# HKUST-Aerial-Robotics/VINS-Mono

Measured on AMD Instinct MI355X. Metric: sliding-window BA solves/sec (Estimator::optimization: 8-iteration dogleg solve + marginalization), higher is better.
Workload: dtype f64; 1 GPU; batch of 256 independent EuRoC-shape windows per step and GPU (K=11 frames, ~150 landmarks, 10 IMU factors, ~600 projection factors, 75-dim marginalization prior, max 8 iterations, MARGIN_OLD marginalization); windows resident in HBM; consecutive steps are issued to 16 HIP streams (independent batches in flight); windows_per_gpu=256, batches_in_flight=16, parallelism=independent batches x1 (no collectives)

## Files before the change

vins-mono_amd/csrc/ba_host.hip:

```cpp
#include "vg_range.h"
#include <hip/hip_runtime.h>
#include <algorithm>
#include <chrono>
#include <cmath>
#include <cstdio>
#include <cstdlib>
#include <cstring>
#include <string>
#include <thread>
#include <vector>
#include "ba_layout.h"
#include "vg_handle.h"
#include "../../include/vinsgpu.h"

struct BaFork { hipStream_t aux; hipEvent_t fork, join; };
extern "C" hipError_t ba_launch_solve(const BaLayout& L, const BaLayout* dL, const BaPtrs& P, int rounds, hipStream_t stream,
                                      hipEvent_t* ev, int* kinds, int* n_launches, const BaFork* fk);
typedef int (*BaAllReduce)(void* user, double* buf, size_t count, void* stream);
extern "C" hipError_t ba_launch_solve_big(const BaLayout& L, const BaLayout* dL, const BaPtrs& P, int rounds, int slack, hipStream_t stream,
                                          BaAllReduce allreduce, void* user, int* hook_rc, hipEvent_t* ev, int* kinds, int* n_launches);
extern "C" hipError_t ba_launch_eval_factors(const BaLayout& L, const BaLayout* dL, const BaPtrs& P, double* proj_r, double* proj_J,
                                            double* imu_r, double* imu_J, double* prior_r, hipStream_t stream);
extern "C" const char* ba_failed_launch();
extern "C" hipError_t ba_prepare_launch();
// ... 215 lines not shown
        else { L.l_pmap = 0; L.l_pinv = o; o += up(L.R, 4) / 2; }
        if (L.big) { L.l_di = o; o += up(L.Rc + 1, 2); L.l_cz = o; o += 6 * 96; }
        L.l_Sg = 0;
        if (L.big) { L.l_Sg = oo; oo += up((L.Rc + 1) * (L.Rc + 2) / 2, 2); }
        L.lds_solve = o * 8;
        bigm_doubles = ob;
        if (!L.big && L.Rc + 10 - 64 > 32) { h->err = "solve kernel: more column tasks than three wavefronts"; return VG_ERR_UNSUPPORTED; }
        if (!L.big && 36 * ldc < std::max(std::max(L.RcPad * 33, 2 * SV_NT), std::max(9 * L.K, 162))) { h->err = "solve kernel: scratch does not fit the coupling-row ring"; return VG_ERR_UNSUPPORTED; }
        if (L.lds_solve > 160 * 1024) { h->err = "solve kernel LDS carve exceeds 160 KB"; return VG_ERR_UNSUPPORTED; }
        const int nib = std::min(std::min(L.K - 1, BA_IMU_BATCH), L.igs);
        L.lds_lin = 8 * std::max(up(nib * 225, 2) + nib * 480, 5 * L.Ncap);
        L.lds_pro = 8 * BA_NW * (L.imu_info ? 512 : 256);
        if (8 * L.Ncap * L.Ncap <= 128 * 1024) L.lds_pro = std::max(L.lds_pro, 8 * L.Ncap * L.Ncap);
        if (L.lds_lin > 128 * 1024) { h->err = "prior too large for the linearisation kernel"; return VG_ERR_UNSUPPORTED; }
        {
            static const bool env_off = getenv("VG_BA_FUSED") && !strcmp(getenv("VG_BA_FUSED"), "0");
            const bool off = env_off && !h->ba.no_env;
            static const int env_min = getenv("VG_BA_FUSED_MIN") ? atoi(getenv("VG_BA_FUSED_MIN")) : 32;
            const int la_min_windows = h->ba.fused_min >= 0 ? (h->ba.fused_min ? h->ba.fused_min : 1 << 30) : (env_min ? env_min : 1 << 30);
            const int npair = L.Kp * (L.Kp - 1) / 2;
            const int avail = (160 * 1024 - 8192 - 512) / 8;
            const int nstl = up(7 * L.Kp + 9 * L.K + 8, 2);
            int chf = (int)((avail - nstl - npair * 90 - 34 - (64 + 82 + 8 * 80) / 2) / 34.0);
            chf = std::min(chf & ~1, 512);
            L.la_on = (!off && L.nwin >= la_min_windows && !L.big && !L.e && !L.t && L.Kp <= 13 && chf >= 96 && (L.Fcap + chf - 17) / (chf - 16) <= 62) ? 1 : 0;
            L.la_chf = chf; L.la_chq = chf - 16;
            L.la_P = up(chf * 33, 2);
            L.la_key = L.la_P + up(npair * 90, 2);
            L.la_x = up(L.la_key + (2 * chf + 64 + 82 + 8 * 80 + 1) / 2 + 2, 2);
            L.lds_linacc = (L.la_x + nstl) * 8;
        }
        {
            static const int env_max = getenv("VG_BA_SOLVE_W8_BELOW") ? atoi(getenv("VG_BA_SOLVE_W8_BELOW")) : -1;
            const int below = (env_max >= 0 && !h->ba.no_env) ? env_max : 32;
            L.sv_w8 = (!L.big && L.nwin < below) ? 1 : 0;
            L.l_wd8 = L.lds_solve / 8;
            L.lds_solve_w8 = L.lds_solve + 8 * L.RcPad * 33;
            if (L.lds_solve_w8 > 160 * 1024) L.sv_w8 = 0;
        }
    }
    if (L.big) {
        const int nt = (L.Rc + 1 + 15) / 16;
        L.nts = nt * (nt + 1) / 2;
        const int ntri = L.Rc * (L.Rc + 1) / 2;
        L.rb1_T = up(ntri + L.Rc, 2);
        L.rb1_scal = L.rb1_T + up((L.Rc + 1) * (L.Rc + 2) / 2, 2);
        L.rb1_len = L.rb1_scal + RB1_NSCAL;
    }
    int o = 0;
    L.io_hdr = o; o += BA_HDR_INTS;
    L.io_lm_start = o; o += L.Lcap;
    L.io_lm_fbeg = o; o += L.Lcap + 8;
    L.io_fac_i = o; o += L.Fcap;
// ... 42 lines not shown
    L.so_gn = o; o += L.Rpad + L.Lcap;
    L.so_yl = o; o += L.Lcap;
    L.so_lsc = o; o += L.Lcap;
    L.so_xp = 0;
    if (!L.big) { L.so_xp = o; o += up(9 * L.K, 4) * L.ldc; }
    if (L.big) {
        L.so_bigm = o; o += up(bigm_doubles, 8);
        L.so_dgl = o; o += 2 * L.Lcap;
        L.so_gtl = o; o += 2 * L.Lcap;
    }
    {
        int b = 0;
        L.bo_Sp = b; b += up(L.Rc * (L.Rc + 1) / 2, 2);
        L.bo_gp = b; b += L.RcPad;
        L.bo_h = b; b += L.Lcap;
        L.bo_b = b; b += L.Lcap;
        L.bo_Wt = b; b += L.RcPad * L.Lcap;
        L.bo_imuJ = b; b += (L.K - 1) * 512;
        L.bo_pr = b; b += L.Ncap;
        L.bo_gpr = b; b += L.Ncap;
        L.buf_stride = up(b, 8);
    }
    L.so_buf = o; o += 2 * L.buf_stride;
    L.sstride = up(o, 8);
    L.pl_off = (int)((sizeof(BaLayout) + 255) / 256 * 256);
    L.pl_n = L.big ? 0 : L.Rc * (L.Rc + 1) / 2 + L.Rpad + 2 * 81 * L.K;
    o = 0;
    L.oo_pose = o; o += up(7 * L.Kp, 2);
    L.oo_sb = o; o += up(9 * L.K, 2);
    L.oo_ex = o; o += 8;
    L.oo_td = o; o += 2;
    L.oo_lam = o; o += L.Lcap;
    L.oo_sum = o; o += BA_SUM_DOUBLES;
    L.oo_trace = o; o += 5 * VG_MAX_ITERS + 16;
    L.ostride = up(o, 8);
    L.oi_stride = up(4 + VG_MAX_ITERS, 8);
    L.mcap = up(6 * L.K + 9 * 2 + 6 + 1, 8);
    if (L.mcap > 256) { h->err = "kept dimension of the marginalization beyond the kernel's tables"; return VG_ERR_UNSUPPORTED; }
    const int mcap = L.mcap;
    L.mo_J0 = 0;
    L.mo_r0 = mcap * mcap;
    L.mo_x0 = L.mo_r0 + mcap;
    L.mo_stride = up(L.mo_x0 + (L.K + 4) * 9, 8);
    L.mi_stride = up(8 + 2 * (L.K + 4) + 16, 8);
    L.mg_posmax = up(mcap + 15 + L.Lcap, 2);
    {
// ... 1144 lines not shown
```

vins-mono_amd/csrc/ba_layout.h:

```cpp
#pragma once

#ifndef BA_NT
#define BA_NT 512
#endif
#define BA_NW (BA_NT / 64)
#ifndef SV_NT
#define SV_NT 256
#endif
#define SV_NW (SV_NT / 64)
#define SV_WG_PER_CU (SV_NT <= 256 ? 2 : 1)
#define BA_LIN_NT 256
#define BA_ACC_NT 256
#define BA_MAX_K 13
#define BA_MAX_K_LARGE 40
#define BA_MARG_LDS_INTS 400
#ifndef BA_IMU_BATCH
#define BA_IMU_BATCH 16
#endif
#ifndef BA_IMU_GROUP
#define BA_IMU_GROUP 2
#endif
#define BA_IMU_STRIDE 472
#define BA_OBS_STRIDE 8
#define BA_SUM_DOUBLES 16
#define BA_HDR_INTS 16

enum { H_L = 0, H_F, H_NPRIOR, H_NBLK, H_MAXIT, H_NCHUNK, H_MARGIN, H_STATUS, H_MARGMODE };

enum {
    C_IT = 0, C_NACC, C_NINV, C_TERM, C_STATUS, C_RADIUS, C_MU, C_MUSOLVED, C_REUSE, C_COST, C_XNORM, C_ALPHA, C_GTN2,
    C_GNN2, C_GTGN, C_DNORM, C_MODEL, C_CUR, C_PENDING, C_DONE, C_STEPNORM, C_XNORMC, C_INITCOST, C_SCALED, C_QCAM,
    C_PHASE, C_GNN2C, C_GTGNC, C_STEP2C, C_XN2C,
    C_T0,
    C_TIMEDOUT,
    C_NCTL = 32
};

enum { RB1_COST = 0, RB1_GTL2, RB1_LAM2, RB1_STEP2, RB1_NBIG, RB1_NSCAL = 8 };
enum { RB2_GNN2 = 0, RB2_GTGN, RB2_QL, RB2_NONFIN };
#define BA_BIG_LM_BLOCKS 32
#define BA_BIG_ZERO_BLOCKS 8
#define RB2_LEN (4 * BA_BIG_LM_BLOCKS)

enum { V_G = 0, V_SC, V_DG, V_GT, V_GN, V_U, V_Y, V_T, V_DI, V_NVEC };
struct alignas(16) AsmPlanEntry { int dst, base, imu, cols; };

struct BaLayout {
    int nwin, K, Kp, e, t;
// ... 8 lines not shown
        io_pair_ptr, io_task_list, io_imu_valid, io_pb_kind, io_pb_idx, io_pb_col, io_pb_off, io_pb_x0off, istride;
    int do_pose, do_sb, do_ex, do_td, do_lam, do_obs, do_imu, do_par, dstride;
    int po_x0, po_r0, po_J0, pld, pstride;
    int so_ctl, so_part, so_x, so_lam;
    int so_imuU, so_Hp, so_rec;
    int so_J0t;
    int so_sc, so_sl, so_dg, so_gt, so_gn;
    int so_yl, so_lsc;
    int so_xp;
    int so_buf, buf_stride;
    int bo_Sp, bo_gp, bo_h, bo_b, bo_Wt, bo_imuJ, bo_pr, bo_gpr;
    int sstride;
    int oo_pose, oo_sb, oo_ex, oo_td, oo_lam, oo_sum, oo_trace, ostride;
    int oi_stride;
    int mo_J0, mo_r0, mo_x0, mo_stride;
    int mi_stride;
    int ms_stride;
    int mcap, mg_ld, mg_posmax, mg_cs, mg_lds_bytes;
    int l_S, l_XC, l_D, l_E, l_dinv, l_vec, l_red, l_wd, l_z, l_pmap, ldc, lds_solve;
    int l_ring, l_pinv;
    int pl_off, pl_n;
    int lds_lin, lds_pro;
    int la_on, la_chq, la_chf, la_P, la_key, la_x, lds_linacc;
    int sv_w8;
    int l_wd8, lds_solve_w8;
    int pro_split;
    int big;
    int so_bigm;
    int l_di, l_cz;
    int l_Sg;
    int so_dgl, so_gtl;
    int rb1_len, rb1_T, rb1_scal;
    int nts;
};

struct BaPtrs {
    int* iarr;
    double* din;
    double* scr;
    double* out;
    int* iout;
    double* mout;
    int* miout;
    double* mscr;
    double* rb1;
    double* rb2;
// ... 5 lines not shown
```

vins-mono_amd/csrc/ba_pipeline.hip:

```cpp
#include <hip/hip_runtime.h>
#include <vector>
#include <mutex>
#include <cstring>
#include <cstdlib>
#include "ba_layout.h"
#include "ba_factors.h"
#include "../../include/vinsgpu.h"

extern __shared__ __attribute__((aligned(16))) char bp_smem[];

#ifdef BA_SOLVE_W8_TU
#undef BA_PROFILE_DETAIL
#undef BA_DEBUG_DUMP
namespace vg_w8 {
#endif

#define NOINL __device__ __noinline__
#define AS_LDS(p) ((lds_d*)(p))
#define AS_LDS_C(p) ((const lds_d*)(p))
#define AS_GLB(p) ((glb_d*)(p))
#define AS_GLB_C(p) ((const glb_d*)(p))
#define AS_GLB_CI(p) ((const glb_i*)(p))
template <bool BIG> struct MovT { typedef lds_d D; typedef lds_i I; };
template <> struct MovT<true> { typedef glb_d D; typedef glb_i I; };
// ... 43 lines not shown
    for (int k_ = c.tid; k_ < L.lds_solve / 8; k_ += SV_NT) g_dbg[(slot) * DBG_SLOT + k_] = LDSB[k_]; \
    if ((slot) >= 2) for (int k_ = c.tid; k_ < 9 * L.K * L.ldc; k_ += SV_NT) g_dbg[5 * DBG_SLOT + k_] = m.xp[k_]; \
    __syncthreads(); } } while (0)
#else
#define DBG_DUMP(slot)
#endif
enum { PF_JUDGE = 0, PF_ASM, PF_DG, PF_BUILD, PF_CHAIN, PF_SCHUR, PF_CHOL, PF_BACK, PF_CBACK, PF_LMY, PF_NORMS, PF_CAND, PF_TAIL };


struct Ctx {
    const BaLayout* Lp;
    const int* hdr;
    const int* ia;
    const double* di;
    const double* pri;
    double* sc;
    int tid, lane, wave;
    int nL, nF, nprior, nblk;
    double focal, tr, row, gnorm;
};

DEV BaLayout layout_load(const BaLayout* Lp) { return const_load(Lp); }

DEV void ctx_init(Ctx& c, const BaLayout* Lp, const BaPtrs& P, int w) {
    const BaLayout L = layout_load(Lp);
    c.Lp = Lp;
    c.ia = P.iarr + (size_t)w * L.istride;
    c.hdr = c.ia + L.io_hdr;
    c.di = P.din + (size_t)w * L.dstride;
    c.sc = P.scr + (size_t)w * L.sstride;
    c.pri = P.pri + (size_t)w * L.pstride;
    c.tid = threadIdx.x; c.lane = c.tid & 63; c.wave = c.tid >> 6;
    c.nL = uni(c.hdr[H_L]); c.nF = uni(c.hdr[H_F]); c.nprior = uni(c.hdr[H_NPRIOR]); c.nblk = uni(c.hdr[H_NBLK]);
    c.focal = uni(c.di[L.do_par + P_FOCAL]); c.tr = uni(c.di[L.do_par + P_TR]); c.row = uni(c.di[L.do_par + P_ROW]);
    c.gnorm = uni(c.di[L.do_par + P_GNORM]);
}

DEV double block_sum(double* red, int nw, int lane, int wave, double v) {
    v = wave_sum_all(v);
    __syncthreads();
    if (lane == 0) red[wave] = v;
    __syncthreads();
    double s = 0.0;
    for (int w = 0; w < nw; ++w) s += red[w];
    return uni(s);
}
DEV void block_sum2(double* red, int nw, int lane, int wave, double& a, double& b) {
    a = wave_sum_all(a);
    b = wave_sum_all(b);
    __syncthreads();
    if (lane == 0) { red[wave] = a; red[nw + wave] = b; }
    __syncthreads();
    double s = 0.0, t = 0.0;
    for (int w = 0; w < nw; ++w) { s += red[w]; t += red[nw + w]; }
// ... 207 lines not shown
#pragma unroll
            for (int k = 0; k < 15; ++k) A[c.lane * 15 + k] = a[k];
        }
        __builtin_amdgcn_wave_barrier();
        glb_d* Uo = AS_GLB(c.sc + L.so_imuU + f * 225);
        if (c.lane < 15) {
            const int j = c.lane;
            double x[15];
#pragma unroll
            for (int i = 14; i >= 0; --i) {
                double s = (i == j) ? 1.0 : 0.0;
#pragma unroll
                for (int k = 14; k > i; --k) s -= (k <= j) ? A[i * 15 + k] * x[k] : 0.0;
                x[i] = (i <= j) ? s / A[i * 15 + i] : 0.0;
            }
#pragma unroll
            for (int i = 0; i < 15; ++i) Uo[i * 15 + j] = x[i];
        }
        __builtin_amdgcn_wave_barrier();
    }
    __syncthreads();
}

#ifndef BA_SOLVE_W8_TU
extern "C" __global__ __launch_bounds__(BA_NT) void ba_prologue_kernel(const BaLayout* __restrict__ Lp, BaPtrs P) {
    const BaLayout& L = *Lp;
    Ctx c;
    ctx_init(c, Lp, P, blockIdx.x);
    double* x = c.sc + L.so_x;
    DP_DECL;
    const bool all = gridDim.y == 1;
    const int part = blockIdx.y, nI = (L.K - 1 + BA_NW - 1) / BA_NW;
    if (all || part == 0)
    {
        double* out = P.out + (size_t)blockIdx.x * L.ostride;
        int* iout = P.iout + (size_t)blockIdx.x * L.oi_stride;
        int* miout = P.miout + (size_t)blockIdx.x * L.mi_stride;
        for (int k = c.tid; k < L.ostride; k += BA_NT) out[k] = 0.0;
        for (int k = c.tid; k < L.oi_stride; k += BA_NT) iout[k] = 0;
        for (int k = c.tid; k < L.mi_stride; k += BA_NT) miout[k] = 0;
    }
    if (all || part == 0) {
        for (int k = c.tid; k < 7 * L.Kp; k += BA_NT) x[k] = c.di[L.do_pose + k];
        for (int k = c.tid; k < 9 * L.K; k += BA_NT) x[7 * L.Kp + k] = c.di[L.do_sb + k];
        if (c.tid < 7) x[7 * L.Kp + 9 * L.K + c.tid] = c.di[L.do_ex + c.tid];
        if (c.tid == 7) x[7 * L.Kp + 9 * L.K + 7] = c.di[L.do_td];
        for (int k = c.tid; k < c.nL; k += BA_NT) c.sc[L.so_lam + k] = c.di[L.do_lam + k];
        if (c.tid < C_NCTL) {
            double v = 0.0;
            if (c.tid == C_RADIUS) v = 1e4;
            if (c.tid == C_MU || c.tid == C_MUSOLVED) v = 1e-8;
            if (c.tid == C_T0) v = (double)wall_clock64();
            c.sc[L.so_ctl + c.tid] = v;
        }
    }
    DP_ADD(40);
    if (all || (part >= 1 && part <= nI)) {
        const int fbeg = all ? 0 : (part - 1) * BA_NW, fend = all ? L.K - 1 : part * BA_NW;
        if (L.imu_info) imu_sqrt_info_ref(c, fbeg, fend);
        else imu_sqrt_info(c, fbeg, fend);
    }
    DP_ADD(41);
    if (c.nprior && (all || part > nI)) {
        const bool do_copy = all || part == nI + 1, do_prod = all || part == nI + 2;
        const int n = c.nprior;
        const double* J0 = c.pri + L.po_J0;
        double* Hp = c.sc + L.so_Hp;
        if (do_copy) {
            double* J0t = c.sc + L.so_J0t;
            for (int wk = c.tid; wk < n * n; wk += BA_NT) { const int r = wk / n, cc = wk % n; J0t[cc * L.Ncap + r] = J0[r * L.pld + cc]; }
        }
        __syncthreads();
        DP_ADD(42);
        if (!do_prod) {
        } else if ((size_t)n * n * 8 <= (size_t)L.lds_pro) {
            double* J0s = LDSB;
            for (int wk = c.tid; wk < n * n; wk += BA_NT) J0s[wk] = J0[(wk / n) * L.pld + wk % n];
// ... 292 lines not shown
struct ProjIn {
    double pi[7], pj[7], oi[8], oj[8], ex[8];
    double lam;
    int i, j, l;
};
DEV void proj_fetch(const Ctx& c, int f, const double* x_, const double* lam_, ProjIn& p) {
    const BaLayout& L = *c.Lp;
    const glb_i* ia = AS_GLB_CI(c.ia);
    const glb_d* x = AS_GLB_C(x_);
    const glb_d* obs = AS_GLB_C(c.di + L.do_obs);
    p.i = ia[L.io_fac_i + f];
    p.j = ia[L.io_fac_j + f];
    p.l = ia[L.io_fac_lm + f];
    const int oi = ia[L.io_fac_oi + f], oj = ia[L.io_fac_oj + f];
#pragma unroll
    for (int k = 0; k < 7; ++k) { p.pi[k] = x[7 * p.i + k]; p.pj[k] = x[7 * p.j + k]; }
#pragma unroll
    for (int k = 0; k < 8; ++k) {
        p.oi[k] = obs[oi * BA_OBS_STRIDE + k];
        p.oj[k] = obs[oj * BA_OBS_STRIDE + k];
        p.ex[k] = x[7 * L.Kp + 9 * L.K + k];
    }
    p.lam = AS_GLB_C(lam_)[p.l];
}
DEV void proj_fetch_staged(const Ctx& c, int f, const lds_d* xs, const double* lam_, ProjIn& p) {
    const BaLayout& L = *c.Lp;
    const glb_i* ia = AS_GLB_CI(c.ia);
    const glb_d* obs = AS_GLB_C(c.di + L.do_obs);
    p.i = ia[L.io_fac_i + f];
    p.j = ia[L.io_fac_j + f];
    p.l = ia[L.io_fac_lm + f];
    const int oi = ia[L.io_fac_oi + f], oj = ia[L.io_fac_oj + f];
#pragma unroll
    for (int k = 0; k < 8; ++k) {
        p.oi[k] = obs[oi * BA_OBS_STRIDE + k];
        p.oj[k] = obs[oj * BA_OBS_STRIDE + k];
    }
    p.lam = AS_GLB_C(lam_)[p.l];
#pragma unroll
    for (int k = 0; k < 7; ++k) { p.pi[k] = xs[7 * p.i + k]; p.pj[k] = xs[7 * p.j + k]; }
#pragma unroll
    for (int k = 0; k < 8; ++k) p.ex[k] = xs[7 * L.Kp + 9 * L.K + k];
}
DEV void proj_jac(const Ctx& c, const ProjIn& p, double* r, double* Ji, double* Jj, double* Jex,
                  double* Jl, double* Jtd) {
    const BaLayout& L = *c.Lp;
    if (L.t) {
        if (L.e) proj_eval<true, true, true>(p.pi, p.pj, p.ex, p.lam, p.oi, p.oj, p.ex[7], c.focal, c.tr, c.row, r, Ji, Jj, Jex, Jl, Jtd);
        else proj_eval<true, true, false>(p.pi, p.pj, p.ex, p.lam, p.oi, p.oj, p.ex[7], c.focal, c.tr, c.row, r, Ji, Jj, Jex, Jl, Jtd);
    } else {
        if (L.e) proj_eval<false, true, true>(p.pi, p.pj, p.ex, p.lam, p.oi, p.oj, 0.0, c.focal, c.tr, c.row, r, Ji, Jj, Jex, Jl, Jtd);
        else proj_eval<false, true, false>(p.pi, p.pj, p.ex, p.lam, p.oi, p.oj, 0.0, c.focal, c.tr, c.row, r, Ji, Jj, Jex, Jl, Jtd);
    }
}

NOINL double proj_linearize(const Ctx& c_in, int f, const double* x, const double* lam, double* recs) {
    const Ctx c = c_in;
    const BaLayout L = *c.Lp;
    ProjIn p;
    proj_fetch(c, f, x, lam, p);
    double r[2], Ji[12], Jj[12], Jex[12], Jl[2], Jtd[2];
    proj_jac(c, p, r, Ji, Jj, Jex, Jl, Jtd);
    const double s = r[0] * r[0] + r[1] * r[1];
    const double sq = sqrt(1.0 / (1.0 + s));
    glb_d* rec = AS_GLB(recs) + (size_t)AS_GLB_CI(c.ia)[L.io_fac_slot + f] * L.REC;
// ... 260 lines not shown
    const int bx = rest % L.nba, w = (rest / L.nba) * 8 + xcd;
    if (w >= L.nwin) return;
    Ctx c;
    ctx_init(c, Lp, P, w);
    const double* ctl = c.sc + L.so_ctl;
    if (ctl[C_DONE] != 0.0) return;
    const int which = ((int)ctl[C_CUR]) ^ (ctl[C_PENDING] != 0.0 ? 1 : 0);
    double* buf = lin_buf(c, which);
    const double* recs = c.sc + L.so_rec;
    __shared__ double part[7 * 36 + 4];
    if (bx < L.Kp) { diag_pose_task(c, bx, recs, buf + L.bo_Sp, buf + L.bo_gp, part); return; }
    const int ng = L.e + L.t;
    if (ng && bx == L.Kp) { global_task(c, recs, buf + L.bo_Sp, buf + L.bo_gp, part); return; }
    const int g = (bx - L.Kp - (ng ? 1 : 0)) * (BA_ACC_NT / 64) + c.wave;
    const int nother = L.ntask - L.Kp - ng * (ng + 1) / 2;
    if (g < nother) owner_task(c, c.ia[L.io_task_list + g], c.lane, recs, buf + L.bo_Sp, buf + L.bo_gp);
    else {
        const int l = (g - nother) * 64 + c.lane;
        if (l < L.Lcap) landmark_task(c, l, recs, buf);
    }
}
#endif

#define LA_NT BA_NT
#define LA_RS 33
#define LA_NPW 6
#define LA_MAXP 13
#define LA_QCAP 80
static_assert(LA_QCAP <= 128, "the pair prefix of ba_linacc_proj_kernel takes two pairs per lane of one wavefront");
#define LA_PAIR 90
DEV int wave_scan_incl(int v) {
    v += __builtin_amdgcn_update_dpp(0, v, 0x111, 0xF, 0xF, true);
    v += __builtin_amdgcn_update_dpp(0, v, 0x112, 0xF, 0xF, true);
    v += __builtin_amdgcn_update_dpp(0, v, 0x114, 0xF, 0xF, true);
    v += __builtin_amdgcn_update_dpp(0, v, 0x118, 0xF, 0xF, true);
    const int r0 = __builtin_amdgcn_readlane(v, 15), r1 = __builtin_amdgcn_readlane(v, 31), r2 = __builtin_amdgcn_readlane(v, 47);
    const int row = (int)(threadIdx.x & 63) >> 4;
    return v + (row > 0 ? r0 : 0) + (row > 1 ? r1 : 0) + (row > 2 ? r2 : 0);
}
DEV int la_pair_q(int i, int j, int Kp) { const int d = j - i; return (d - 1) * Kp - (d - 1) * d / 2 + i; }
__device__ __forceinline__ void linacc_body(const BaLayout* __restrict__ Lp, const BaPtrs& P) {
    const BaLayout L = layout_load(Lp);
    Ctx c;
    ctx_init(c, Lp, P, blockIdx.x);
    const double* ctl = c.sc + L.so_ctl;
    if (ctl[C_DONE] != 0.0) return;
    const int which = uni(((int)ctl[C_CUR]) ^ (ctl[C_PENDING] != 0.0 ? 1 : 0));
    const double* x = c.sc + L.so_x + which * L.nst;
    const double* lam = c.sc + L.so_lam + which * L.Lcap;
    glb_d* buf = AS_GLB(lin_buf(c, which));
    const glb_i* ia = AS_GLB_CI(c.ia);
    lds_d* rec = AS_LDS(LDSB);
    lds_d* Pb = AS_LDS(LDSB + L.la_P);
    lds_i* key = (lds_i*)(LDSB + L.la_key);
    lds_i* lstart = key + L.la_chf;
    lds_i* posx = lstart + 64;
    lds_i* pstart = posx + L.la_chf;
    lds_i* wcnt = pstart + LA_QCAP + 2;
    __shared__ double red[2 * (LA_NT / 64)];
    const int Kp = L.Kp, npair = Kp * (Kp - 1) / 2, chq = L.la_chq;
    const int nL = c.nL;
    DP_DECL;
    {
        double share = 0.0;
        if (c.nprior > 0) {
            if (c.nprior * c.nprior <= 12 * LA_NT && 4 * L.Ncap <= 4 * LA_NT && (c.nprior * (c.nprior + 1) + 2 + 5 * L.Ncap) <= L.la_P)
                share = prior_staged(c, L, x, lin_buf(c, which) + L.bo_pr, lin_buf(c, which) + L.bo_gpr, LDSB);
            else
                share = prior_pass(c, x, lin_buf(c, which) + L.bo_pr, lin_buf(c, which) + L.bo_gpr, LDSB);
        }
        DP_ADD(23);
        share += imu_pass<true>(c, x, lin_buf(c, which) + L.bo_imuJ, 0, L.K - 1);
        const double tot_imu = block_sum(red, LA_NT / 64, c.lane, c.wave, share);
        for (int g = c.tid; g < L.nbl - L.nbf; g += LA_NT) c.sc[L.so_part + L.nbf + g] = g == 0 ? tot_imu : 0.0;
        __syncthreads();
        DP_ADD(22);
    }
    lds_d* xs = AS_LDS(LDSB + L.la_x);
    for (int k = c.tid; k < 7 * L.Kp + 9 * L.K + 8; k += LA_NT) xs[k] = AS_GLB_C(x)[k];
    const int nchunk = nL > 0 ? uni(ia[L.io_lm_fbeg + nL - 1] / chq + 1) : 0;
    for (int t = c.tid; t < nL; t += LA_NT) {
        const int cl = ia[L.io_lm_fbeg + t] / chq;
        if (t == 0 || ia[L.io_lm_fbeg + t - 1] / chq != cl) lstart[cl] = t;
    }
    if (c.tid == 0) lstart[nchunk] = nL;
    for (int e = c.tid; e < npair * LA_PAIR; e += LA_NT) Pb[e] = 0.0;
    const bool pair_wave = c.wave < LA_NPW;
    __syncthreads();
    DP_ADD(24);
    int pidx[4];
#pragma unroll
    for (int reg = 0; reg < 4; ++reg) {
        const int row = (c.lane >> 4) + 4 * reg, col = c.lane & 15;
        int idx = -1;
        if (row < 6) {
            if (col <= row) idx = row * (row + 1) / 2 + col;
            else if (col == 13) idx = 78 + row;
        } else if (row < 12) {
            if (col < 6) idx = 42 + (row - 6) * 6 + col;
            else if (col <= row && col < 12) idx = 21 + (row - 6) * (row - 5) / 2 + (col - 6);
            else if (col == 13) idx = 84 + (row - 6);
        }
        pidx[reg] = idx;
    }
    double cost = 0.0;
    for (int ch = 0; ch < nchunk; ++ch) {
        const int l0 = lstart[ch], l1 = lstart[ch + 1];
        const int f0 = ia[L.io_lm_fbeg + l0], f1 = ia[L.io_lm_fbeg + l1];
        const int nf = uni(f1 - f0);
        if (nf > L.la_chf) __builtin_trap();
        ProjIn pin;
        int q = -1, rank = 0;
        if (c.tid < nf) {
            proj_fetch_staged(c, f0 + c.tid, xs, lam, pin);
            q = la_pair_q(pin.i, pin.j, Kp);
        }
        for (int e = c.tid; e < (LA_NT / 64) * LA_QCAP; e += LA_NT) wcnt[e] = 0;
        __syncthreads();
        DP_ADD(45);
        {
            const unsigned long long act = __ballot(q >= 0);
            unsigned long long same = act;
#pragma unroll
            for (int b = 0; b < 7; ++b) {
                const bool bit = q >= 0 && ((q >> b) & 1);
                const unsigned long long mb = __ballot(bit);
                same &= bit ? mb : ~mb;
            }
            const unsigned long long lt = (1ull << c.lane) - 1ull;
            rank = __popcll(same & lt);
            if (q >= 0 && rank == 0) wcnt[c.wave * LA_QCAP + q] = __popcll(same);
        }
        __syncthreads();
        if (c.wave == 0) {
            int cw0[LA_NT / 64], cw1[LA_NT / 64];
            const int p0 = c.lane, p1 = c.lane + 64;
#pragma unroll
            for (int w = 0; w < LA_NT / 64; ++w) {
                cw0[w] = p0 < npair ? wcnt[w * LA_QCAP + p0] : 0;
                cw1[w] = p1 < npair ? wcnt[w * LA_QCAP + p1] : 0;
            }
            int t0 = 0, t1 = 0;
#pragma unroll
            for (int w = 0; w < LA_NT / 64; ++w) { const int a = cw0[w], b = cw1[w]; cw0[w] = t0; cw1[w] = t1; t0 += a; t1 += b; }
            const int i0 = wave_scan_incl(t0);
            const int tot0 = __builtin_amdgcn_readlane(i0, 63);
            const int i1 = wave_scan_incl(t1) + tot0;
            if (p0 < npair) {
                pstart[p0 + 1] = i0;
#pragma unroll
                for (int w = 0; w < LA_NT / 64; ++w) wcnt[w * LA_QCAP + p0] = i0 - t0 + cw0[w];
            }
            if (p1 < npair) {
                pstart[p1 + 1] = i1;
#pragma unroll
                for (int w = 0; w < LA_NT / 64; ++w) wcnt[w * LA_QCAP + p1] = i1 - t1 + cw1[w];
            }
            if (c.lane == 0) pstart[0] = 0;
        }
        __syncthreads();
        DP_ADD(46);
        if (c.tid < nf) {
            const int pos = wcnt[c.wave * LA_QCAP + q] + rank;
            double r[2], Ji[12], Jj[12], Jl[2];
            proj_eval<false, true, false>(pin.pi, pin.pj, pin.ex, pin.lam, pin.oi, pin.oj, 0.0, c.focal, c.tr, c.row, r, Ji, Jj, nullptr, Jl, nullptr);
            const double s = r[0] * r[0] + r[1] * r[1];
            const double sq = sqrt(1.0 / (1.0 + s));
            lds_d* qr = rec + pos * LA_RS;
#pragma unroll
            for (int k = 0; k < 6; ++k) {
                qr[k] = sq * Ji[k]; qr[16 + k] = sq * Ji[6 + k];
                qr[6 + k] = sq * Jj[k]; qr[22 + k] = sq * Jj[6 + k];
            }
            qr[12] = sq * Jl[0]; qr[28] = sq * Jl[1];
            qr[13] = sq * r[0]; qr[29] = sq * r[1];
            key[c.tid] = pin.i * 16 + pin.j;
            posx[c.tid] = pos;
            cost += log1p(s);
        }
        __syncthreads();
        DP_ADD(25);
        if (pair_wave) {
            double4_t acc[LA_MAXP];
#pragma unroll
            for (int k = 0; k < LA_MAXP; ++k) acc[k] = (double4_t){0, 0, 0, 0};
            const int k4 = c.lane >> 4, col = c.lane & 15;
            const int xo = (k4 & 1) * 16 + col;
            const int hi = k4 >> 1;
            const bool incol = col < 14;
#pragma unroll
            for (int k = 0; k < LA_MAXP; ++k) {
                const int qk = c.wave + LA_NPW * k;
                if (qk >= npair) continue;
                const int pb0 = uni(pstart[qk]), pe0 = uni(pstart[qk + 1]);
                DP_ADD(29);
                for (int e = pb0; e < pe0; e += 4) {
                    const int f0r = e + hi, f1r = e + 2 + hi;
                    const double v0 = (f0r < pe0 && incol) ? rec[f0r * LA_RS + xo] : 0.0;
                    const double v1 = (f1r < pe0 && incol) ? rec[f1r * LA_RS + xo] : 0.0;
                    acc[k] = __builtin_amdgcn_mfma_f64_16x16x4f64(v0, v0, acc[k], 0, 0, 0);
                    if (e + 2 < pe0) acc[k] = __builtin_amdgcn_mfma_f64_16x16x4f64(v1, v1, acc[k], 0, 0, 0);
                }
                DP_ADD(30);
            }
#pragma unroll
            for (int k = 0; k < LA_MAXP; ++k) {
                if (c.wave + LA_NPW * k >= npair) continue;
                lds_d* pb = Pb + (c.wave + LA_NPW * k) * LA_PAIR;
                double old4[4];
#pragma unroll
                for (int reg = 0; reg < 4; ++reg) old4[reg] = (ch > 0 && pidx[reg] >= 0) ? pb[pidx[reg]] : 0.0;
#pragma unroll
                for (int reg = 0; reg < 4; ++reg)
                    if (pidx[reg] >= 0) pb[pidx[reg]] = old4[reg] + acc[k][reg];
            }
            DP_ADD(26);
        } else {
            for (int t = c.tid - LA_NPW * 64; t < l1 - l0; t += LA_NT - LA_NPW * 64) {
                const int l = l0 + t;
                glb_d* Wt = buf + L.bo_Wt + l;
                const size_t ldw = L.Lcap;
                const int fb = ia[L.io_lm_fbeg + l] - f0, fe = ia[L.io_lm_fbeg + l + 1] - f0;
                double h = 0.0, b = 0.0, wi[6] = {0, 0, 0, 0, 0, 0};
                const int anchor = fb < fe ? key[fb] >> 4 : -1;
                int jn = 0;
                for (int f = fb; f < fe; ++f) {
                    const lds_d* q = rec + posx[f] * LA_RS;
                    const int j = key[f] & 15;
                    const double l0v = q[12], l1v = q[28];
                    double v[6];
#pragma unroll
                    for (int k = 0; k < 6; ++k) v[k] = q[6 + k] * l0v + q[22 + k] * l1v;
                    h += l0v * l0v + l1v * l1v;
                    b += l0v * q[13] + l1v * q[29];
#pragma unroll
                    for (int k = 0; k < 6; ++k) wi[k] += q[k] * l0v + q[16 + k] * l1v;
                    for (; jn < j; ++jn) {
                        if (jn == anchor) continue;
#pragma unroll
                        for (int k = 0; k < 6; ++k) Wt[(size_t)(6 * jn + k) * ldw] = 0.0;
                    }
#pragma unroll
                    for (int k = 0; k < 6; ++k) Wt[(size_t)(6 * j + k) * ldw] = v[k];
                    jn = j + 1;
                }
                for (; jn < Kp; ++jn) {
                    if (jn == anchor) continue;
#pragma unroll
                    for (int k = 0; k < 6; ++k) Wt[(size_t)(6 * jn + k) * ldw] = 0.0;
                }
                if (anchor >= 0) {
// ... 2953 lines not shown
```

vins-mono_amd/csrc/vg_target.h:

```cpp
#pragma once
#include <hip/hip_runtime.h>
#include <stdint.h>

#ifndef VINS_SIMT
typedef __attribute__((address_space(3))) double lds_d;
typedef __attribute__((address_space(3))) int lds_i;
typedef __attribute__((address_space(1))) double glb_d;
typedef __attribute__((address_space(1))) int glb_i;
typedef __attribute__((address_space(1))) uint8_t glb_u8;
typedef __attribute__((address_space(1))) uint32_t glb_u32;
typedef __attribute__((address_space(1))) uint16_t glb_u16;
typedef uint32_t vg_u32_a2 __attribute__((aligned(2)));
typedef __attribute__((address_space(1))) const vg_u32_a2 glb_u32_a2;
#define VG_WAVES_PER_EU(n) __attribute__((amdgpu_waves_per_eu(n, n)))
typedef const __attribute__((address_space(4))) char* vg_kernarg_ptr;
#define BA_WALL_HZ 1e8
#define VG_KEEP_ALIVE(p) asm volatile("" :: "v"(p))
__device__ __forceinline__ int vg_mul24(int a, int b) { return __mul24(a, b); }
__device__ __forceinline__ int uni(int v) { return __builtin_amdgcn_readfirstlane(v); }
__device__ __forceinline__ double uni(double v) {
    return __hiloint2double(__builtin_amdgcn_readfirstlane(__double2hiint(v)), __builtin_amdgcn_readfirstlane(__double2loint(v)));
}
template <typename T>
__device__ __forceinline__ T const_load(const T* p) {
    T v;
    __builtin_memcpy(&v, (const __attribute__((address_space(4))) void*)p, sizeof(T));
    return v;
}
__device__ __forceinline__ uint4 vg_load16_unaligned(const glb_u8* p) {
    typedef unsigned int nv4 __attribute__((ext_vector_type(4), aligned(1)));
    typedef __attribute__((address_space(1))) const nv4 glb_nv4;
    const nv4 t4 = *(glb_nv4*)p;
    uint4 v;
    v.x = t4.x; v.y = t4.y; v.z = t4.z; v.w = t4.w;
    return v;
}
__device__ __forceinline__ int4 vg_load_int4(const void* p) {
    typedef int nv4 __attribute__((ext_vector_type(4)));
    typedef __attribute__((address_space(1))) const nv4 glb_nv4;
    const nv4 t4 = *(glb_nv4*)p;
// ... 22 lines not shown
    typedef short s2 __attribute__((ext_vector_type(2)));
    return __builtin_amdgcn_sdot2(__builtin_bit_cast(s2, a), __builtin_bit_cast(s2, b), c, false);
}
__device__ __forceinline__ int vg_sdot2_keep(unsigned a, unsigned b, int c) {
    int r;
    asm("v_dot2_i32_i16 %0, %1, %2, %3" : "=v"(r) : "v"(a), "v"(b), "v"(c));
    return r;
}

#else
typedef double lds_d;
typedef int lds_i;
typedef double glb_d;
typedef int glb_i;
typedef uint8_t glb_u8;
typedef uint32_t glb_u32;
typedef uint16_t glb_u16;
typedef uint32_t vg_u32_a2 __attribute__((aligned(2)));
typedef const vg_u32_a2 glb_u32_a2;
#define VG_WAVES_PER_EU(n)
typedef const char* vg_kernarg_ptr;
#define BA_WALL_HZ 1e9
#define VG_KEEP_ALIVE(p) ((void)(p))
inline int vg_mul24(int a, int b) { return a * b; }
inline int uni(int v) { return v; }
inline double uni(double v) { return v; }
template <typename T> inline T const_load(const T* p) { return *p; }
inline uint4 vg_load16_unaligned(const glb_u8* p) { uint4 v; __builtin_memcpy(&v, p, 16); return v; }
inline int4 vg_load_int4(const void* p) { int4 v; __builtin_memcpy(&v, p, 16); return v; }
template <int Q> inline unsigned vg_byte_pair(unsigned hi, unsigned lo) {
    const unsigned long long v = ((unsigned long long)hi << 32) | lo;
    return (unsigned)((v >> (8 * Q)) & 255u) | ((unsigned)((v >> (8 * (Q + 1))) & 255u) << 16);
}
template <unsigned SEL> inline unsigned vg_perm(unsigned hi, unsigned lo) {
    const unsigned long long v = ((unsigned long long)hi << 32) | lo;
    unsigned r = 0;
    for (int i = 0; i < 4; ++i) {
        const unsigned sel = (SEL >> (8 * i)) & 255u;
        if (sel < 8) r |= (unsigned)((v >> (8 * sel)) & 255u) << (8 * i);
        else if (sel != 0x0Cu) { fprintf(stderr, "simt: unmodelled v_perm_b32 selector 0x%x\n", sel); abort(); }
    }
    return r;
}
inline unsigned vg_pk_add(unsigned a, unsigned b) { return ((a + b) & 0xffffu) | (((a >> 16) + (b >> 16)) << 16); }
inline unsigned vg_pk_sub(unsigned a, unsigned b) { return ((a - b) & 0xffffu) | (((a >> 16) - (b >> 16)) << 16); }
inline unsigned vg_pk_mad(unsigned a, unsigned short k, unsigned c) { return (((a & 0xffffu) * k + (c & 0xffffu)) & 0xffffu) | (((a >> 16) * k + (c >> 16)) << 16); }
// ... 5 lines not shown
```

Before: 192,100 solves/s.

## Precompute per-window factor sort plan in prologue and reuse across linearisation iterations

New measurement: 190,200 solves/s. About the same (-1.0%).

```diff
diff --git a/vins-mono_amd/csrc/ba_host.hip b/vins-mono_amd/csrc/ba_host.hip
--- a/vins-mono_amd/csrc/ba_host.hip
+++ b/vins-mono_amd/csrc/ba_host.hip
@@ -261,13 +261,15 @@
             const int avail = (160 * 1024 - 8192 - 512) / 8;
             const int nstl = up(7 * L.Kp + 9 * L.K + 8, 2);
             int chf = (int)((avail - nstl - npair * 90 - 34 - (64 + 82 + 8 * 80) / 2) / 34.0);
+            chf = std::min(chf, (int)((avail - nstl - L.Lcap - npair * 90 - 34 - (2 * 66) / 2) / 33.5));
             chf = std::min(chf & ~1, 512);
             L.la_on = (!off && L.nwin >= la_min_windows && !L.big && !L.e && !L.t && L.Kp <= 13 && chf >= 96 && (L.Fcap + chf - 17) / (chf - 16) <= 62) ? 1 : 0;
             L.la_chf = chf; L.la_chq = chf - 16;
             L.la_P = up(chf * 33, 2);
             L.la_key = L.la_P + up(npair * 90, 2);
-            L.la_x = up(L.la_key + (2 * chf + 64 + 82 + 8 * 80 + 1) / 2 + 2, 2);
-            L.lds_linacc = (L.la_x + nstl) * 8;
+            L.la_x = up(L.la_key + (chf + 2 * 66 + 1) / 2 + 2, 2);
+            L.la_lam = L.la_x + nstl;
+            L.lds_linacc = (L.la_lam + L.Lcap) * 8;
         }
         {
             static const int env_max = getenv("VG_BA_SOLVE_W8_BELOW") ? atoi(getenv("VG_BA_SOLVE_W8_BELOW")) : -1;
@@ -356,6 +358,17 @@
         L.buf_stride = up(b, 8);
     }
     L.so_buf = o; o += 2 * L.buf_stride;
+    L.so_plan = L.fp_pr = L.fp_pos = L.fp_ijl = L.fp_obs = 0;
+    if (!L.big && !L.e && !L.t && L.Kp <= 13 && L.la_chf >= 96) {
+        const int nchmax = (L.Fcap + L.la_chf - 17) / (L.la_chf - 16) + 1;
+        L.so_plan = o;
+        int io = FP_FIXED;
+        L.fp_pr = io; io += nchmax * LA_NPW * 16;
+        L.fp_pos = io; io += L.Fcap;
+        L.fp_ijl = io; io += L.Fcap;
+        o += up(io, 4) / 2;
+        L.fp_obs = o; o += 4 * L.Fcap;
+    }
     L.sstride = up(o, 8);
     L.pl_off = (int)((sizeof(BaLayout) + 255) / 256 * 256);
     L.pl_n = L.big ? 0 : L.Rc * (L.Rc + 1) / 2 + L.Rpad + 2 * 81 * L.K;
diff --git a/vins-mono_amd/csrc/ba_layout.h b/vins-mono_amd/csrc/ba_layout.h
--- a/vins-mono_amd/csrc/ba_layout.h
+++ b/vins-mono_amd/csrc/ba_layout.h
@@ -24,6 +24,8 @@
 #define BA_OBS_STRIDE 8
 #define BA_SUM_DOUBLES 16
 #define BA_HDR_INTS 16
+enum { FP_NCHUNK = 0, FP_LSTART = 2, FP_FBEG = 68, FP_FIXED = 136 };
+#define LA_NPW 6
 
 enum { H_L = 0, H_F, H_NPRIOR, H_NBLK, H_MAXIT, H_NCHUNK, H_MARGIN, H_STATUS, H_MARGMODE };
 
@@ -78,6 +80,7 @@
     int pl_off, pl_n;
     int lds_lin, lds_pro;
     int la_on, la_chq, la_chf, la_P, la_key, la_x, lds_linacc;
+    int so_plan, fp_pr, fp_pos, fp_ijl, fp_obs, la_lam;
     int sv_w8;
     int l_wd8, lds_solve_w8;
     int pro_split;
diff --git a/vins-mono_amd/csrc/ba_pipeline.hip b/vins-mono_amd/csrc/ba_pipeline.hip
--- a/vins-mono_amd/csrc/ba_pipeline.hip
+++ b/vins-mono_amd/csrc/ba_pipeline.hip
@@ -89,14 +89,17 @@
 
 DEV BaLayout layout_load(const BaLayout* Lp) { return const_load(Lp); }
 
-DEV void ctx_init(Ctx& c, const BaLayout* Lp, const BaPtrs& P, int w) {
-    const BaLayout L = layout_load(Lp);
-    c.Lp = Lp;
+DEV void ctx_pointers(Ctx& c, const BaLayout& L, const BaPtrs& P, int w) {
     c.ia = P.iarr + (size_t)w * L.istride;
     c.hdr = c.ia + L.io_hdr;
     c.di = P.din + (size_t)w * L.dstride;
     c.sc = P.scr + (size_t)w * L.sstride;
     c.pri = P.pri + (size_t)w * L.pstride;
+}
+DEV void ctx_init(Ctx& c, const BaLayout* Lp, const BaPtrs& P, int w) {
+    const BaLayout L = layout_load(Lp);
+    c.Lp = Lp;
+    ctx_pointers(c, L, P, w);
     c.tid = threadIdx.x; c.lane = c.tid & 63; c.wave = c.tid >> 6;
     c.nL = uni(c.hdr[H_L]); c.nF = uni(c.hdr[H_F]); c.nprior = uni(c.hdr[H_NPRIOR]); c.nblk = uni(c.hdr[H_NBLK]);
     c.focal = uni(c.di[L.do_par + P_FOCAL]); c.tr = uni(c.di[L.do_par + P_TR]); c.row = uni(c.di[L.do_par + P_ROW]);
@@ -350,6 +353,116 @@
     __syncthreads();
 }
 
+#define LA_NT BA_NT
+#define LA_RS 33
+#define LA_MAXP 13
+#define LA_QCAP 80
+static_assert(LA_QCAP <= 128, "the pair prefix of ba_linacc_proj_kernel takes two pairs per lane of one wavefront");
+#define LA_PAIR 90
+DEV int wave_scan_incl(int v) {
+    v += __builtin_amdgcn_update_dpp(0, v, 0x111, 0xF, 0xF, true);
+    v += __builtin_amdgcn_update_dpp(0, v, 0x112, 0xF, 0xF, true);
+    v += __builtin_amdgcn_update_dpp(0, v, 0x114, 0xF, 0xF, true);
+    v += __builtin_amdgcn_update_dpp(0, v, 0x118, 0xF, 0xF, true);
+    const int r0 = __builtin_amdgcn_readlane(v, 15), r1 = __builtin_amdgcn_readlane(v, 31), r2 = __builtin_amdgcn_readlane(v, 47);
+    const int row = (int)(threadIdx.x & 63) >> 4;
+    return v + (row > 0 ? r0 : 0) + (row > 1 ? r1 : 0) + (row > 2 ? r2 : 0);
+}
+DEV int la_pair_q(int i, int j, int Kp) { const int d = j - i; return (d - 1) * Kp - (d - 1) * d / 2 + i; }
+
+DEV void build_factor_plan(const Ctx& c, const BaLayout& L) {
+    const glb_i* ia = AS_GLB_CI(c.ia);
+    glb_i* pl = (glb_i*)(c.sc + L.so_plan);
+    glb_d* po = AS_GLB(c.sc + L.fp_obs);
+    const glb_d* obs = AS_GLB_C(c.di + L.do_obs);
+    lds_i* lstart = (lds_i*)LDSB;
+    lds_i* pstart = lstart + 66;
+    lds_i* wcnt = pstart + LA_QCAP + 2;
+    const int Kp = L.Kp, npair = Kp * (Kp - 1) / 2, chq = L.la_chq;
+    const int nL = c.nL;
+    const int nchunk = nL > 0 ? uni(ia[L.io_lm_fbeg + nL - 1] / chq + 1) : 0;
+    for (int t = c.tid; t < nL; t += BA_NT) {
+        const int cl = ia[L.io_lm_fbeg + t] / chq;
+        if (t == 0 || ia[L.io_lm_fbeg + t - 1] / chq != cl) lstart[cl] = t;
+    }
+    if (c.tid == 0) { lstart[nchunk] = nL; pl[FP_NCHUNK] = nchunk; }
+    __syncthreads();
+    if (c.tid <= nchunk) {
+        const int l = lstart[c.tid];
+        pl[FP_LSTART + c.tid] = l;
+        pl[FP_FBEG + c.tid] = ia[L.io_lm_fbeg + l];
+    }
+    for (int ch = 0; ch < nchunk; ++ch) {
+        const int f0 = uni(ia[L.io_lm_fbeg + lstart[ch]]), f1 = uni(ia[L.io_lm_fbeg + lstart[ch + 1]]);
+        const int nf = f1 - f0;
+        if (nf > L.la_chf) __builtin_trap();
+        const int f = f0 + c.tid;
+        int q = -1, rank = 0, fi = 0, fj = 0;
+        if (c.tid < nf) {
+            fi = ia[L.io_fac_i + f];
+            fj = ia[L.io_fac_j + f];
+            q = la_pair_q(fi, fj, Kp);
+        }
+        for (int e = c.tid; e < (BA_NT / 64) * LA_QCAP; e += BA_NT) wcnt[e] = 0;
+        __syncthreads();
+        {
+            const unsigned long long act = __ballot(q >= 0);
+            unsigned long long same = act;
+#pragma unroll
+            for (int b = 0; b < 7; ++b) {
+                const bool bit = q >= 0 && ((q >> b) & 1);
+                const unsigned long long mb = __ballot(bit);
+                same &= bit ? mb : ~mb;
+            }
+            const unsigned long long lt = (1ull << c.lane) - 1ull;
+            rank = __popcll(same & lt);
+            if (q >= 0 && rank == 0) wcnt[c.wave * LA_QCAP + q] = __popcll(same);
+        }
+        __syncthreads();
+        if (c.wave == 0) {
+            int cw0[BA_NT / 64], cw1[BA_NT / 64];
+            const int p0 = c.lane, p1 = c.lane + 64;
+#pragma unroll
+            for (int w = 0; w < BA_NT / 64; ++w) {
+                cw0[w] = p0 < npair ? wcnt[w * LA_QCAP + p0] : 0;
+                cw1[w] = p1 < npair ? wcnt[w * LA_QCAP + p1] : 0;
+            }
+            int t0 = 0, t1 = 0;
+#pragma unroll
+            for (int w = 0; w < BA_NT / 64; ++w) { const int a = cw0[w], b = cw1[w]; cw0[w] = t0; cw1[w] = t1; t0 += a; t1 += b; }
+            const int i0 = wave_scan_incl(t0);
+            const int tot0 = __builtin_amdgcn_readlane(i0, 63);
+            const int i1 = wave_scan_incl(t1) + tot0;
+            if (p0 < npair) {
+                pstart[p0 + 1] = i0;
+#pragma unroll
+                for (int w = 0; w < BA_NT / 64; ++w) wcnt[w * LA_QCAP + p0] = i0 - t0 + cw0[w];
+            }
+            if (p1 < npair) {
+                pstart[p1 + 1] = i1;
+#pragma unroll
+                for (int w = 0; w < BA_NT / 64; ++w) wcnt[w * LA_QCAP + p1] = i1 - t1 + cw1[w];
+            }
+            if (c.lane == 0) pstart[0] = 0;
+        }
+        __syncthreads();
+        if (c.tid < nf) {
+            const int oi = ia[L.io_fac_oi + f], oj = ia[L.io_fac_oj + f];
+            pl[L.fp_pos + f] = wcnt[c.wave * LA_QCAP + q] + rank;
+            pl[L.fp_ijl + f] = fi << 4 | fj | ia[L.io_fac_lm + f] << 8;
+            po[f] = obs[oi * BA_OBS_STRIDE];
+            po[L.Fcap + f] = obs[oi * BA_OBS_STRIDE + 1];
+            po[2 * L.Fcap + f] = obs[oj * BA_OBS_STRIDE];
+            po[3 * L.Fcap + f] = obs[oj * BA_OBS_STRIDE + 1];
+        }
+        for (int e = c.tid; e < LA_NPW * 16; e += BA_NT) {
+            const int k = e & 15, qk = (e >> 4) + LA_NPW * k;
+            pl[L.fp_pr + ch * (LA_NPW * 16) + e] = (k < LA_MAXP && qk < npair) ? pstart[qk] | pstart[qk + 1] << 16 : 0;
+        }
+        __syncthreads();
+    }
+}
+
 #ifndef BA_SOLVE_W8_TU
 extern "C" __global__ __launch_bounds__(BA_NT) void ba_prologue_kernel(const BaLayout* __restrict__ Lp, BaPtrs P) {
     const BaLayout& L = *Lp;
@@ -381,6 +494,7 @@
             if (c.tid == C_T0) v = (double)wall_clock64();
             c.sc[L.so_ctl + c.tid] = v;
         }
+        if (L.la_on) build_factor_plan(c, layout_load(Lp));
     }
     DP_ADD(40);
     if (all || (part >= 1 && part <= nI)) {
@@ -719,25 +833,6 @@
         p.ex[k] = x[7 * L.Kp + 9 * L.K + k];
     }
     p.lam = AS_GLB_C(lam_)[p.l];
-}
-DEV void proj_fetch_staged(const Ctx& c, int f, const lds_d* xs, const double* lam_, ProjIn& p) {
-    const BaLayout& L = *c.Lp;
-    const glb_i* ia = AS_GLB_CI(c.ia);
-    const glb_d* obs = AS_GLB_C(c.di + L.do_obs);
-    p.i = ia[L.io_fac_i + f];
-    p.j = ia[L.io_fac_j + f];
-    p.l = ia[L.io_fac_lm + f];
-    const int oi = ia[L.io_fac_oi + f], oj = ia[L.io_fac_oj + f];
-#pragma unroll
-    for (int k = 0; k < 8; ++k) {
-        p.oi[k] = obs[oi * BA_OBS_STRIDE + k];
-        p.oj[k] = obs[oj * BA_OBS_STRIDE + k];
-    }
-    p.lam = AS_GLB_C(lam_)[p.l];
-#pragma unroll
-    for (int k = 0; k < 7; ++k) { p.pi[k] = xs[7 * p.i + k]; p.pj[k] = xs[7 * p.j + k]; }
-#pragma unroll
-    for (int k = 0; k < 8; ++k) p.ex[k] = xs[7 * L.Kp + 9 * L.K + k];
 }
 DEV void proj_jac(const Ctx& c, const ProjIn& p, double* r, double* Ji, double* Jj, double* Jex,
                   double* Jl, double* Jtd) {
@@ -1044,44 +1139,15 @@
 }
 #endif
 
-#define LA_NT BA_NT
-#define LA_RS 33
-#define LA_NPW 6
-#define LA_MAXP 13
-#define LA_QCAP 80
-static_assert(LA_QCAP <= 128, "the pair prefix of ba_linacc_proj_kernel takes two pairs per lane of one wavefront");
-#define LA_PAIR 90
-DEV int wave_scan_incl(int v) {
-    v += __builtin_amdgcn_update_dpp(0, v, 0x111, 0xF, 0xF, true);
-    v += __builtin_amdgcn_update_dpp(0, v, 0x112, 0xF, 0xF, true);
-    v += __builtin_amdgcn_update_dpp(0, v, 0x114, 0xF, 0xF, true);
-    v += __builtin_amdgcn_update_dpp(0, v, 0x118, 0xF, 0xF, true);
-    const int r0 = __builtin_amdgcn_readlane(v, 15), r1 = __builtin_amdgcn_readlane(v, 31), r2 = __builtin_amdgcn_readlane(v, 47);
-    const int row = (int)(threadIdx.x & 63) >> 4;
-    return v + (row > 0 ? r0 : 0) + (row > 1 ? r1 : 0) + (row > 2 ? r2 : 0);
-}
-DEV int la_pair_q(int i, int j, int Kp) { const int d = j - i; return (d - 1) * Kp - (d - 1) * d / 2 + i; }
 __device__ __forceinline__ void linacc_body(const BaLayout* __restrict__ Lp, const BaPtrs& P) {
-    const BaLayout L = layout_load(Lp);
+    BaLayout L = layout_load(Lp);
     Ctx c;
     ctx_init(c, Lp, P, blockIdx.x);
     const double* ctl = c.sc + L.so_ctl;
     if (ctl[C_DONE] != 0.0) return;
     const int which = uni(((int)ctl[C_CUR]) ^ (ctl[C_PENDING] != 0.0 ? 1 : 0));
     const double* x = c.sc + L.so_x + which * L.nst;
-    const double* lam = c.sc + L.so_lam + which * L.Lcap;
-    glb_d* buf = AS_GLB(lin_buf(c, which));
-    const glb_i* ia = AS_GLB_CI(c.ia);
-    lds_d* rec = AS_LDS(LDSB);
-    lds_d* Pb = AS_LDS(LDSB + L.la_P);
-    lds_i* key = (lds_i*)(LDSB + L.la_key);
-    lds_i* lstart = key + L.la_chf;
-    lds_i* posx = lstart + 64;
-    lds_i* pstart = posx + L.la_chf;
-    lds_i* wcnt = pstart + LA_QCAP + 2;
     __shared__ double red[2 * (LA_NT / 64)];
-    const int Kp = L.Kp, npair = Kp * (Kp - 1) / 2, chq = L.la_chq;
-    const int nL = c.nL;
     DP_DECL;
     {
         double share = 0.0;
@@ -1098,14 +1164,27 @@
         __syncthreads();
         DP_ADD(22);
     }
+    L = layout_load(vg_refetch(Lp));
+    ctx_pointers(c, L, P, blockIdx.x);
+    const glb_d* xg = AS_GLB_C(c.sc + L.so_x + which * L.nst);
+    const glb_d* lamg = AS_GLB_C(c.sc + L.so_lam + which * L.Lcap);
+    glb_d* buf = AS_GLB(c.sc + L.so_buf + which * L.buf_stride);
+    const glb_i* ia = AS_GLB_CI(c.ia);
+    lds_d* rec = AS_LDS(LDSB);
+    lds_d* Pb = AS_LDS(LDSB + L.la_P);
+    const int Kp = L.Kp, npair = Kp * (Kp - 1) / 2;
+    const int nL = c.nL;
+    lds_i* pk = (lds_i*)(LDSB + L.la_key);
+    lds_i* lstart = pk + L.la_chf;
+    lds_i* fbeg = lstart + 66;
+    const glb_i* pl = (const glb_i*)(c.sc + L.so_plan);
+    const glb_d* po = AS_GLB_C(c.sc + L.fp_obs);
     lds_d* xs = AS_LDS(LDSB + L.la_x);
-    for (int k = c.tid; k < 7 * L.Kp + 9 * L.K + 8; k += LA_NT) xs[k] = AS_GLB_C(x)[k];
-    const int nchunk = nL > 0 ? uni(ia[L.io_lm_fbeg + nL - 1] / chq + 1) : 0;
-    for (int t = c.tid; t < nL; t += LA_NT) {
-        const int cl = ia[L.io_lm_fbeg + t] / chq;
-        if (t == 0 || ia[L.io_lm_fbeg + t - 1] / chq != cl) lstart[cl] = t;
-    }
-    if (c.tid == 0) lstart[nchunk] = nL;
+    lds_d* lams = AS_LDS(LDSB + L.la_lam);
+    for (int k = c.tid; k < 7 * L.Kp + 9 * L.K + 8; k += LA_NT) xs[k] = xg[k];
+    for (int k = c.tid; k < nL; k += LA_NT) lams[k] = lamg[k];
+    const int nchunk = uni(pl[FP_NCHUNK]);
+    if (c.tid <= nchunk) { lstart[c.tid] = pl[FP_LSTART + c.tid]; fbeg[c.tid] = pl[FP_FBEG + c.tid]; }
     for (int e = c.tid; e < npair * LA_PAIR; e += LA_NT) Pb[e] = 0.0;
     const bool pair_wave = c.wave < LA_NPW;
     __syncthreads();
@@ -1128,64 +1207,21 @@
     double cost = 0.0;
     for (int ch = 0; ch < nchunk; ++ch) {
         const int l0 = lstart[ch], l1 = lstart[ch + 1];
-        const int f0 = ia[L.io_lm_fbeg + l0], f1 = ia[L.io_lm_fbeg + l1];
-        const int nf = uni(f1 - f0);
+        const int f0 = uni(fbeg[ch]), nf = uni(fbeg[ch + 1]) - f0;
         if (nf > L.la_chf) __builtin_trap();
-        ProjIn pin;
-        int q = -1, rank = 0;
+        int prr = 0;
+        if (pair_wave) prr = pl[L.fp_pr + (ch * LA_NPW + c.wave) * 16 + (c.lane & 15)];
         if (c.tid < nf) {
-            proj_fetch_staged(c, f0 + c.tid, xs, lam, pin);
-            q = la_pair_q(pin.i, pin.j, Kp);
-        }
-        for (int e = c.tid; e < (LA_NT / 64) * LA_QCAP; e += LA_NT) wcnt[e] = 0;
-        __syncthreads();
-        DP_ADD(45);
-        {
-            const unsigned long long act = __ballot(q >= 0);
-            unsigned long long same = act;
-#pragma unroll
-            for (int b = 0; b < 7; ++b) {
-                const bool bit = q >= 0 && ((q >> b) & 1);
-                const unsigned long long mb = __ballot(bit);
-                same &= bit ? mb : ~mb;
-            }
-            const unsigned long long lt = (1ull << c.lane) - 1ull;
-            rank = __popcll(same & lt);
-            if (q >= 0 && rank == 0) wcnt[c.wave * LA_QCAP + q] = __popcll(same);
-        }
-        __syncthreads();
-        if (c.wave == 0) {
-            int cw0[LA_NT / 64], cw1[LA_NT / 64];
-            const int p0 = c.lane, p1 = c.lane + 64;
-#pragma unroll
-            for (int w = 0; w < LA_NT / 64; ++w) {
-                cw0[w] = p0 < npair ? wcnt[w * LA_QCAP + p0] : 0;
-                cw1[w] = p1 < npair ? wcnt[w * LA_QCAP + p1] : 0;
-            }
-            int t0 = 0, t1 = 0;
-#pragma unroll
-            for (int w = 0; w < LA_NT / 64; ++w) { const int a = cw0[w], b = cw1[w]; cw0[w] = t0; cw1[w] = t1; t0 += a; t1 += b; }
-            const int i0 = wave_scan_incl(t0);
-            const int tot0 = __builtin_amdgcn_readlane(i0, 63);
-            const int i1 = wave_scan_incl(t1) + tot0;
-            if (p0 < npair) {
-                pstart[p0 + 1] = i0;
-#pragma unroll
-                for (int w = 0; w < LA_NT / 64; ++w) wcnt[w * LA_QCAP + p0] = i0 - t0 + cw0[w];
-            }
-            if (p1 < npair) {
-                pstart[p1 + 1] = i1;
-#pragma unroll
-                for (int w = 0; w < LA_NT / 64; ++w) wcnt[w * LA_QCAP + p1] = i1 - t1 + cw1[w];
-            }
-            if (c.lane == 0) pstart[0] = 0;
-        }
-        __syncthreads();
-        DP_ADD(46);
-        if (c.tid < nf) {
-            const int pos = wcnt[c.wave * LA_QCAP + q] + rank;
+            const int f = f0 + c.tid;
+            const int pos = pl[L.fp_pos + f], ijl = pl[L.fp_ijl + f];
+            const double oi[2] = {po[f], po[L.Fcap + f]}, oj[2] = {po[2 * L.Fcap + f], po[3 * L.Fcap + f]};
+            const int fi = (ijl >> 4) & 15, fj = ijl & 15;
+            double pi[7], pj[7], ex[7];
+#pragma unroll
+            for (int k = 0; k < 7; ++k) { pi[k] = xs[7 * fi + k]; pj[k] = xs[7 * fj + k]; ex[k] = xs[7 * L.Kp + 9 * L.K + k]; }
+            const double lamv = lams[ijl >> 8];
             double r[2], Ji[12], Jj[12], Jl[2];
-            proj_eval<false, true, false>(pin.pi, pin.pj, pin.ex, pin.lam, pin.oi, pin.oj, 0.0, c.focal, c.tr, c.row, r, Ji, Jj, nullptr, Jl, nullptr);
+            proj_eval<false, true, false>(pi, pj, ex, lamv, oi, oj, 0.0, c.focal, c.tr, c.row, r, Ji, Jj, nullptr, Jl, nullptr);
             const double s = r[0] * r[0] + r[1] * r[1];
             const double sq = sqrt(1.0 / (1.0 + s));
             lds_d* qr = rec + pos * LA_RS;
@@ -1196,8 +1232,7 @@
             }
             qr[12] = sq * Jl[0]; qr[28] = sq * Jl[1];
             qr[13] = sq * r[0]; qr[29] = sq * r[1];
-            key[c.tid] = pin.i * 16 + pin.j;
-            posx[c.tid] = pos;
+            pk[c.tid] = pos << 8 | (ijl & 255);
             cost += log1p(s);
         }
         __syncthreads();
@@ -1214,7 +1249,8 @@
             for (int k = 0; k < LA_MAXP; ++k) {
                 const int qk = c.wave + LA_NPW * k;
                 if (qk >= npair) continue;
-                const int pb0 = uni(pstart[qk]), pe0 = uni(pstart[qk + 1]);
+                const int pr = __builtin_amdgcn_readlane(prr, k);
+                const int pb0 = pr & 0xffff, pe0 = pr >> 16;
                 DP_ADD(29);
                 for (int e = pb0; e < pe0; e += 4) {
                     const int f0r = e + hi, f1r = e + 2 + hi;
@@ -1244,11 +1280,12 @@
                 const size_t ldw = L.Lcap;
                 const int fb = ia[L.io_lm_fbeg + l] - f0, fe = ia[L.io_lm_fbeg + l + 1] - f0;
                 double h = 0.0, b = 0.0, wi[6] = {0, 0, 0, 0, 0, 0};
-                const int anchor = fb < fe ? key[fb] >> 4 : -1;
+                const int anchor = fb < fe ? (pk[fb] >> 4) & 15 : -1;
                 int jn = 0;
                 for (int f = fb; f < fe; ++f) {
-                    const lds_d* q = rec + posx[f] * LA_RS;
-                    const int j = key[f] & 15;
+                    const int pkf = pk[f];
+                    const lds_d* q = rec + (pkf >> 8) * LA_RS;
+                    const int j = pkf & 15;
                     const double l0v = q[12], l1v = q[28];
                     double v[6];
 #pragma unroll
diff --git a/vins-mono_amd/csrc/vg_target.h b/vins-mono_amd/csrc/vg_target.h
--- a/vins-mono_amd/csrc/vg_target.h
+++ b/vins-mono_amd/csrc/vg_target.h
@@ -16,6 +16,7 @@
 typedef const __attribute__((address_space(4))) char* vg_kernarg_ptr;
 #define BA_WALL_HZ 1e8
 #define VG_KEEP_ALIVE(p) asm volatile("" :: "v"(p))
+template <typename T> __device__ __forceinline__ const T* vg_refetch(const T* p) { asm volatile("" : "+s"(p)); return p; }
 __device__ __forceinline__ int vg_mul24(int a, int b) { return __mul24(a, b); }
 __device__ __forceinline__ int uni(int v) { return __builtin_amdgcn_readfirstlane(v); }
 __device__ __forceinline__ double uni(double v) {
@@ -84,6 +85,7 @@
 typedef const char* vg_kernarg_ptr;
 #define BA_WALL_HZ 1e9
 #define VG_KEEP_ALIVE(p) ((void)(p))
+template <typename T> inline const T* vg_refetch(const T* p) { return p; }
 inline int vg_mul24(int a, int b) { return a * b; }
 inline int uni(int v) { return v; }
 inline double uni(double v) { return v; }
```
